# keurfonluu/stochopy

Measured on AMD Instinct MI355X. Metric: objective-fn evals/sec, higher is better.
Workload: dtype f64

## Files before the change

include/stochopy_hip.h:

```cpp
#ifndef STOCHOPY_HIP_H
#define STOCHOPY_HIP_H

#include <stdint.h>

#ifdef __cplusplus
extern "C" {
#endif

#define SX_ABI_VERSION 1

enum {
    SX_FUN_ACKLEY = 0,
    SX_FUN_GRIEWANK = 1,
    SX_FUN_QUARTIC = 2,
    SX_FUN_RASTRIGIN = 3,
    SX_FUN_ROSENBROCK = 4,
    SX_FUN_SPHERE = 5,
    SX_FUN_STYBLINSKI_TANG = 6,
    SX_FUN_COUNT = 7
};

enum { SX_DE_RAND1BIN = 0, SX_DE_RAND2BIN = 1, SX_DE_BEST1BIN = 2, SX_DE_BEST2BIN = 3 };

enum {
// ... 29 lines not shown
    int64_t gbidx;
    double gfit;
    double dx;
    int32_t status;
    int32_t done;
    int64_t reserved[3];
} sx_state;

typedef struct sx_de_args {
    double *buf0, *buf1;
    double *fit;
    double *candfit;
    double *gbest;
    const double *lower;
    const double *upper;
    sx_state *state;
    double *part_f;
    int64_t *part_i;
    const double *r1;
    const int32_t *donors;
    const int32_t *irand;
    const double *resample;
    int64_t P;
    int64_t ld;
    int64_t row0;
    int32_t n;
    int32_t fun_id;
    int32_t strategy;
    int32_t constraints;
    int32_t rng;
    int32_t maxiter;
    int32_t wide_from;
    int32_t pad;
    double F, CR, xtol, ftol;
    uint32_t key0, key1;
} sx_de_args;

int sx_de_generation(const sx_de_args *a, int finalize, void *stream);

int sx_select_finalize(const double *part_f, const int64_t *part_i, int64_t npart, const double *rows0,
                       const double *rows1, int64_t ld, int n, double *gbest, sx_state *state, int maxiter,
                       double xtol, double ftol, void *stream);

int sx_shard_best(const double *part_f, const int64_t *part_i, int64_t npart, const double *rows0,
                  const double *rows1, int64_t ld, int n, const sx_state *state, int64_t row0, double *record,
                  void *stream);
int sx_gather_finalize(const double *records, int world, int n, double *gbest, sx_state *state, int maxiter,
                       double xtol, double ftol, void *stream);
int sx_de_shard_generation(const struct sx_de_args *a, double *record, void *stream);

typedef struct sx_graph sx_graph;
int sx_de_graph_create(const sx_de_args *a, int ngen, sx_graph **out);
int sx_de_chain_launch(const sx_de_args *a, int parity, int finalize_only, void *stream);
int sx_de_chain_graph_create(const sx_de_args *a, int ngen, int start_parity, sx_graph **out);
int sx_graph_launch(sx_graph *g, void *stream);
int sx_graph_destroy(sx_graph *g);

#define SX_MAX_PEERS 8
#define SX_IPC_HANDLE_BYTES 64
typedef struct sx_xchg_args {
    uint64_t *peer[SX_MAX_PEERS];
    int32_t world, rank;
    int64_t timeout_ticks;
    int32_t *error;
    uint64_t *relay;
    const double *pop0[SX_MAX_PEERS];
    const double *pop1[SX_MAX_PEERS];
    int64_t global_rows, shard_rows;
} sx_xchg_args;
// ... 202 lines not shown
```

stochopy_amd/_lib.py:

```python
import ctypes as C
import os

_HERE = os.path.dirname(os.path.abspath(__file__))
LIB_PATH = os.path.join(_HERE, "lib", "libstochopy_hip.so")

SX_STATUS_NONE = 100
NARROW_DIM, WIDE_DIM = 4096, 262144


def wide_from():
    return int(lib().sx_wide_from())
SX_RNG_HOST, SX_RNG_PHILOX = 0, 1

FUN_IDS = {
    "ackley": 0,
    "griewank": 1,
    "quartic": 2,
    "rastrigin": 3,
    "rosenbrock": 4,
    "sphere": 5,
    "styblinski_tang": 6,
}
DE_STRATEGIES = {"rand1bin": 0, "rand2bin": 1, "best1bin": 2, "best2bin": 3}
DE_DONORS = {"rand1bin": 3, "rand2bin": 5, "best1bin": 2, "best2bin": 4}

vp = C.c_void_p
i64 = C.c_int64
i32 = C.c_int32
f64 = C.c_double


class SxState(C.Structure):
    _fields_ = [("it", i64), ("gbidx", i64), ("gfit", f64), ("dx", f64), ("status", i32), ("done", i32),
                ("reserved", i64 * 3)]


class SxDeArgs(C.Structure):
    _fields_ = [
        ("buf0", vp), ("buf1", vp), ("fit", vp), ("candfit", vp), ("gbest", vp), ("lower", vp),
        ("upper", vp), ("state", vp), ("part_f", vp), ("part_i", vp), ("r1", vp), ("donors", vp),
        ("irand", vp), ("resample", vp),
        ("P", i64), ("ld", i64), ("row0", i64),
        ("n", i32), ("fun_id", i32), ("strategy", i32), ("constraints", i32), ("rng", i32), ("maxiter", i32),
        ("wide_from", i32), ("pad", i32),
        ("F", f64), ("CR", f64), ("xtol", f64), ("ftol", f64),
        ("key0", C.c_uint32), ("key1", C.c_uint32),
    ]


class SxPsoArgs(C.Structure):
    _fields_ = [
        ("X", vp), ("V", vp), ("pbest", vp), ("pbestfit", vp), ("candfit", vp), ("gbest", vp), ("lower", vp),
        ("upper", vp), ("state", vp), ("part_f", vp), ("part_i", vp), ("r1", vp), ("r2", vp), ("pending_restart", vp),
        ("P", i64), ("ld", i64), ("row0", i64),
        ("n", i32), ("fun_id", i32), ("constraints", i32), ("rng", i32), ("maxiter", i32), ("pad", i32),
        ("w", f64), ("c1", f64), ("c2", f64), ("xtol", f64), ("ftol", f64),
        ("key0", C.c_uint32), ("key1", C.c_uint32),
    ]


SX_MAX_PEERS = 8
SX_IPC_HANDLE_BYTES = 64


class SxXchgArgs(C.Structure):
    _fields_ = [("peer", vp * SX_MAX_PEERS), ("world", i32), ("rank", i32), ("timeout_ticks", i64), ("error", vp),
                ("relay", vp), ("pop0", vp * SX_MAX_PEERS), ("pop1", vp * SX_MAX_PEERS), ("global_rows", i64),
                ("shard_rows", i64)]


class SxCmaState(C.Structure):
    _fields_ = [("it", i64), ("nfev", i64), ("best_row", i64), ("fbest", f64), ("sigma", f64), ("sigma_next", f64),
                ("tmp_coef", f64), ("psnorm", f64), ("status", i32), ("done", i32), ("stop_it", i64),
                ("reserved", f64 * 6)]


class SxVdArgs(C.Structure):
    _fields_ = [
        ("Z", vp), ("ary", vp), ("arx", vp), ("fit", vp), ("xmean", vp), ("xold", vp), ("dx", vp), ("dvec", vp),
        ("vvec", vp), ("vn", vp), ("pc", vp), ("zinj", vp), ("dy", vp), ("w", vp), ("mws", vp), ("mout", vp),
# ... 157 lines not shown
```

stochopy_amd/csrc/sx_de.hip:

```cpp
#define SX_DE_XM 0
#include "sx_de_kernel.hpp"
#include "sx_wide.hpp"

namespace sx {
void *de_chain_kernel(int fun_id, int n, int64_t P, int strategy, int constraints);
void *de_p2p_kernel(int fun_id, int n, int64_t P, int strategy, int constraints);
}

namespace {

int check_args(const sx_de_args *a) {
    SX_REQUIRE(a != nullptr, "sx_de: null args");
    SX_REQUIRE(a->buf0 && a->buf1 && a->fit && a->state && a->part_f && a->part_i, "sx_de: null device pointer");
    SX_REQUIRE(a->P >= 2 && a->P < (int64_t)1 << 31 && a->n >= 1 && a->ld >= a->n, "sx_de: bad shape");
    SX_REQUIRE(a->fun_id >= 0 && a->fun_id < SX_FUN_COUNT, "sx_de: unknown objective");
    SX_REQUIRE(a->strategy >= 0 && a->strategy <= 3, "sx_de: unknown strategy");
    SX_REQUIRE(a->P - 1 >= donors_of(a->strategy), "sx_de: popsize too small for the strategy");
    SX_REQUIRE(a->rng == SX_RNG_HOST || a->rng == SX_RNG_PHILOX, "sx_de: unknown rng mode");
    if (a->rng == SX_RNG_HOST) {
        SX_REQUIRE(a->r1 && a->donors && a->irand, "sx_de: host draws missing");
        SX_REQUIRE(a->constraints == 0 || a->resample, "sx_de: resample block missing");
    }
    SX_REQUIRE(a->constraints == 0 || (a->lower && a->upper), "sx_de: bounds missing");
    return 0;
}

de_kernel_t kernel_for(const sx_de_args *a) {
    return a->rng == SX_RNG_PHILOX ? pick_kernel<SX_RNG_PHILOX, 0>(a->fun_id, a->n, a->P, a->strategy, a->constraints)
                                   : pick_kernel<SX_RNG_HOST, 0>(a->fun_id, a->n, a->P, a->strategy, a->constraints);
}

Geometry geometry(const sx_de_args *a) {
    Geometry g = row_geometry(a->P, a->n, de_wide_from(a));
    if (!is_wide(a->n, de_wide_from(a))) g.lds = (size_t)rows_per_block(a->n) * gen_row_stride(a->n) * sizeof(double);
    return g;
}

}

extern "C" int sx_de_generation(const sx_de_args *a, int finalize, void *stream) {
    if (int rc = check_args(a)) return rc;
    hipStream_t s = (hipStream_t)stream;
    const Geometry g = geometry(a);
    if (is_wide(a->n, de_wide_from(a))) {
        if (int rc = wide_de_launch(a, s)) return rc;
    } else {
        PlanArg plan;
        if (make_plan_arg(a->fun_id, a->n, &plan)) return -1;
        hipLaunchKernelGGL(kernel_for(a), dim3(g.blocks), dim3(g.threads), g.lds, s, (const sx_state *)nullptr,
                           (const double *)nullptr, (const int64_t *)nullptr, (int64_t)g.blocks, *a, plan, 0, 0,
                           sx_xchg_args{});
        SX_LAUNCH_CHECK();
    }
    if (finalize) {
        SX_REQUIRE(a->gbest != nullptr, "sx_de_generation: the separate finalize kernel needs the gbest buffer");
        return sx_select_finalize(a->part_f, a->part_i, g.blocks, a->buf0, a->buf1, a->ld, a->n, a->gbest, a->state,
                                  a->maxiter, a->xtol, a->ftol, stream);
    }
    return 0;
}

extern "C" int sx_de_graph_create(const sx_de_args *a, int ngen, sx_graph **out) {
    if (int rc = check_args(a)) return rc;
    SX_REQUIRE(out != nullptr && ngen >= 1 && a->gbest != nullptr, "sx_de_graph_create: bad arguments");
    SX_REQUIRE(a->rng == SX_RNG_PHILOX, "sx_de_graph_create: graphs need in-kernel (Philox) draws");
    PlanArg plan = {};
    const bool wide = is_wide(a->n, de_wide_from(a));
    if (!wide && make_plan_arg(a->fun_id, a->n, &plan)) return -1;
    const Geometry g = geometry(a);
    sx_graph *gr = new sx_graph();
    SX_HIP(hipGraphCreate(&gr->graph, 0));
    sx_de_args args = *a;
    int zero = 0;
    int64_t npart = g.blocks;
    sx_xchg_args nox = {};
    const void *none = nullptr;
    void *kargs[] = {&none, &none, &none, &npart, &args, &plan, &zero, &zero, &nox};
    hipGraphNode_t prev = nullptr;
    for (int i = 0; i < ngen; ++i) {
        if (wide) {
            if (int rc = wide_de_add_node(gr->graph, &prev, a)) return rc;
        } else {
            hipKernelNodeParams kp = {};
            kp.func = (void *)kernel_for(a);
            kp.gridDim = dim3(g.blocks);
            kp.blockDim = dim3(g.threads);
            kp.sharedMemBytes = (unsigned)g.lds;
            kp.kernelParams = kargs;
            kp.extra = nullptr;
            hipGraphNode_t node;
            SX_HIP(hipGraphAddKernelNode(&node, gr->graph, prev ? &prev : nullptr, prev ? 1 : 0, &kp));
            prev = node;
        }
        if (int rc = add_finalize_node(gr->graph, &prev, a->part_f, a->part_i, g.blocks, a->buf0, a->buf1, a->ld, a->n,
                                       a->gbest, a->state, a->maxiter, a->xtol, a->ftol))
            return rc;
    }
    SX_HIP(hipGraphInstantiate(&gr->exec, gr->graph, nullptr, nullptr, 0));
    *out = gr;
    return 0;
}

extern "C" int sx_de_shard_generation(const sx_de_args *a, double *record, void *stream) {
    SX_REQUIRE(record != nullptr, "sx_de_shard_generation: null record");
    if (int rc = sx_de_generation(a, 0, stream)) return rc;
    return sx_shard_best(a->part_f, a->part_i, (int64_t)geometry(a).blocks, a->buf0, a->buf1, a->ld, a->n, a->state,
                         a->row0, record, stream);
}

static int check_chain(const sx_de_args *a, bool peer_exchange) {
    if (int rc = check_args(a)) return rc;
    SX_REQUIRE(a->rng == SX_RNG_PHILOX, "sx_de_chain: needs in-kernel (Philox) draws");
    SX_REQUIRE(!is_wide(a->n, de_wide_from(a)), "sx_de_chain: rows served by the one-workgroup-per-row kernels (n > wide_from) take the two-kernel path (sx_de_generation)");
    SX_REQUIRE(peer_exchange || geometry(a).blocks <= 512,
               "sx_de_chain: more than 512 workgroup records (use the two-kernel path)");
    return 0;
}

static int chain_launch(const sx_de_args *a, const sx_xchg_args *x, int parity, int finalize_only, void *stream) {
    if (int rc = check_chain(a, x != nullptr)) return rc;
    SX_REQUIRE(parity == 0 || parity == 1, "sx_de_chain_launch: parity must be 0 or 1");
    PlanArg plan;
    if (make_plan_arg(a->fun_id, a->n, &plan)) return -1;
    const Geometry g = geometry(a);
    de_kernel_t kern = (de_kernel_t)(x ? de_p2p_kernel(a->fun_id, a->n, a->P, a->strategy, a->constraints)
                                       : de_chain_kernel(a->fun_id, a->n, a->P, a->strategy, a->constraints));
    const unsigned blocks = finalize_only ? 1u : g.blocks + (x ? 1u : 0u);
    hipLaunchKernelGGL(kern, dim3(blocks), dim3(g.threads), g.lds, (hipStream_t)stream,
                       (const sx_state *)(a->state + parity), (const double *)(a->part_f + (int64_t)parity * g.blocks),
                       (const int64_t *)(a->part_i + (int64_t)parity * g.blocks), (int64_t)g.blocks, *a, plan, parity,
                       finalize_only ? 1 : 0, x ? *x : sx_xchg_args{});
    SX_LAUNCH_CHECK();
    return 0;
}

static int chain_graph_create(const sx_de_args *a, const sx_xchg_args *x, int ngen, int start_parity, sx_graph **out) {
    if (int rc = check_chain(a, x != nullptr)) return rc;
    SX_REQUIRE(out != nullptr && ngen >= 1 && (start_parity == 0 || start_parity == 1),
               "sx_de_chain_graph_create: bad arguments");
    PlanArg plan;
    if (make_plan_arg(a->fun_id, a->n, &plan)) return -1;
    const Geometry g = geometry(a);
    sx_graph *gr = new sx_graph();
    SX_HIP(hipGraphCreate(&gr->graph, 0));
    sx_de_args args = *a;
    sx_xchg_args xa = x ? *x : sx_xchg_args{};
    int mode = 0;
    int64_t npart = g.blocks;
    hipGraphNode_t prev = nullptr;
    for (int i = 0; i < ngen; ++i) {
        int parity = (start_parity + i) & 1;
        const sx_state *sin_pre = a->state + parity;
        const double *pf_pre = a->part_f + (int64_t)parity * npart;
        const int64_t *pi_pre = a->part_i + (int64_t)parity * npart;
        void *kargs[] = {&sin_pre, &pf_pre, &pi_pre, &npart, &args, &plan, &parity, &mode, &xa};
        hipKernelNodeParams kp = {};
        kp.func = x ? de_p2p_kernel(a->fun_id, a->n, a->P, a->strategy, a->constraints)
                    : de_chain_kernel(a->fun_id, a->n, a->P, a->strategy, a->constraints);
        kp.gridDim = dim3(g.blocks + (x ? 1u : 0u));
        kp.blockDim = dim3(g.threads);
        kp.sharedMemBytes = (unsigned)g.lds;
        kp.kernelParams = kargs;
        kp.extra = nullptr;
        hipGraphNode_t node;
        SX_HIP(hipGraphAddKernelNode(&node, gr->graph, prev ? &prev : nullptr, prev ? 1 : 0, &kp));
        prev = node;
    }
    SX_HIP(hipGraphInstantiate(&gr->exec, gr->graph, nullptr, nullptr, 0));
    *out = gr;
    return 0;
}

extern "C" int sx_de_chain_launch(const sx_de_args *a, int parity, int finalize_only, void *stream) {
    return chain_launch(a, nullptr, parity, finalize_only, stream);
}
extern "C" int sx_de_chain_graph_create(const sx_de_args *a, int ngen, int start_parity, sx_graph **out) {
    return chain_graph_create(a, nullptr, ngen, start_parity, out);
}

extern "C" int sx_de_p2p_launch(const sx_de_args *a, const sx_xchg_args *x, int parity, int finalize_only,
                                void *stream) {
    if (int rc = check_xchg_args(x)) return rc;
    return chain_launch(a, x, parity, finalize_only, stream);
}
extern "C" int sx_de_p2p_graph_create(const sx_de_args *a, const sx_xchg_args *x, int ngen, int start_parity,
                                      sx_graph **out) {
    if (int rc = check_xchg_args(x)) return rc;
    return chain_graph_create(a, x, ngen, start_parity, out);
// ... 17 lines not shown
```

stochopy_amd/csrc/sx_de_kernel.hpp:

```cpp
#pragma once
#ifndef SX_DE_XM
#error "define SX_DE_XM (0, 1 or 2) before including sx_de_kernel.hpp"
#endif
#include <type_traits>
#include <vector>

#include "sx_device.hpp"
#include "sx_host.hpp"
#include "sx_rowops.hpp"
#include "sx_xchg.hpp"

namespace sx {
int make_plan_arg(int fun_id, int n, PlanArg *out);
int add_finalize_node(hipGraph_t graph, hipGraphNode_t *prev, const double *part_f, const int64_t *part_i,
                      int64_t npart, const double *rows0, const double *rows1, int64_t ld, int n, double *gbest,
                      sx_state *state, int maxiter, double xtol, double ftol);
int check_xchg_args(const sx_xchg_args *x);
}
using namespace sx;

#if defined(SX_TRACE) && SX_DE_XM == 1
__device__ unsigned long long sx_trace_buf[1024 * 16];
#define SX_TP(k)                                                                              \
    do {                                                                                      \
// ... 103 lines not shown
                        break;
                    }
                    w[u] = ll_load(src + j);
                }
                __hip_atomic_store(dst + j, w[u], __ATOMIC_RELAXED, __HIP_MEMORY_SCOPE_AGENT);
            }
        }
        __builtin_amdgcn_fence(__ATOMIC_RELEASE, "agent");
        __syncthreads();
        if (threadIdx.x == 0)
            __hip_atomic_store(dst + xchg_slot_words(a.n), (uint64_t)tag, __ATOMIC_RELEASE, __HIP_MEMORY_SCOPE_AGENT);
        if (wave != 0) return;
    }
    if (lane == 0) {
        int status = SX_STATUS_NONE;
        if (it >= 2) {
            if (gf <= a.ftol)
                status = 1;
            else if (it >= a.maxiter)
                status = -1;
        }
        sx_state *so = a.state + (mode == 1 ? 2 : 1 - chain_p);
        so->it = it;
        so->gbidx = gi;
        so->gfit = gf;
        so->dx = 0.0;
        so->status = status;
        so->done = status != SX_STATUS_NONE;
        so->reserved[0] = prev_winner;
        so->reserved[1] = winner;
    }
}

constexpr int kStep = 4;

#ifndef SX_DE_NFIX_WAVES
#define SX_DE_NFIX_WAVES 1
#endif
#ifndef SX_DE_WAVE_ROWS_WAVES
#define SX_DE_WAVE_ROWS_WAVES 1
#endif
template <int FUN, int RNG, int XM, int LPR, bool FULL, int NFIX = 0, int STRAT = -1, bool ONEB = false>
__global__ __launch_bounds__(kMaxWavesPerBlock *kWave, (NFIX != 0 && XM <= 1) ? SX_DE_NFIX_WAVES
                                                       : (NFIX == 0 && XM == 0 && STRAT >= 0 && LPR == kWave) ? SX_DE_WAVE_ROWS_WAVES
                                                                                                                 : 1) void de_generation_kernel(const sx_state *const sin_pre,
                                                                                 const double *const pf_pre,
                                                                                 const int64_t *const pi_pre,
                                                                                 const int64_t npart,
                                                                                 const sx_de_args a,
                                                                                 const PlanArg plan,
                                                                                 const int chain_p, const int mode,
                                                                                 const sx_xchg_args x) {
    constexpr bool CHAIN = XM >= 1;
    constexpr bool P2P = XM == 2;
    extern __shared__ __attribute__((aligned(16))) double lds[];
    __shared__ double sf[kMaxRowsPerBlock];
    __shared__ int64_t si[kMaxRowsPerBlock];
    __shared__ double s_gf;
    __shared__ int64_t s_gi;
    __shared__ int s_winner;
    SX_TP(0);
    const int n = NFIX ? NFIX : a.n;
    const int64_t P = a.P, ld = a.ld;
    const RowIds<LPR> id(P, P2P ? 1 : 0);
    const int l = id.l;
    const int64_t rowc = id.rowc;
    double *U = lds + id.slot * gen_row_stride(n);

    const sx_state *sin = (CHAIN && !P2P) ? sin_pre : CHAIN ? a.state + chain_p : a.state;
    constexpr int kRecPerLane = 8;
    double pfv[kRecPerLane];
    using rec_t = typename std::conditional<LPR == kWave, int32_t, int64_t>::type;
    constexpr rec_t kNoRec = LPR == kWave ? (rec_t)INT32_MAX : (rec_t)INT64_MAX;
    rec_t piv[kRecPerLane];
#ifndef SX_CHAIN_REC_WAVE0
#define SX_CHAIN_REC_WAVE0 1
#endif
    if (CHAIN && !P2P && (!SX_CHAIN_REC_WAVE0 || id.wave == 0)) {
        const double *pf = pf_pre;
        const int64_t *pi = pi_pre;
        const int per = (int)((npart + kWave - 1) / kWave);
        const int64_t k0 = (int64_t)id.lane * per;
#pragma unroll
        for (int u = 0; u < kRecPerLane; ++u) {
            const bool in = u < per && k0 + u < npart;
            pfv[u] = in ? pf[k0 + u] : __builtin_huge_val();
            piv[u] = in ? (rec_t)pi[k0 + u] : kNoRec;
        }
    }
    if (P2P && blockIdx.x == 0) {
        p2p_service(a, x, chain_p, mode, npart, sin, LPR == kWave);
        return;
    }
    if (sin->done) {
        if (CHAIN && mode == 1 && threadIdx.x == 0) a.state[2] = *sin;
        return;
    }
    const int64_t it = CHAIN ? sin->it + 1 : sin->it;
    SX_TP(6);

    const uint32_t gen = (uint32_t)(it + 1);
    const double *__restrict__ cur = (it & 1) ? a.buf1 : a.buf0;
    double *__restrict__ nxt = (it & 1) ? a.buf0 : a.buf1;
    const double fold = a.fit[rowc];
    const double *__restrict__ xi = cur + rowc * ld;
    const uint32_t grow = (uint32_t)(a.row0 + rowc);
    const int strategy = STRAT >= 0 ? STRAT : a.strategy;
    const int k = donors_of(strategy);
    const bool repair = STRAT >= 0 ? false : a.constraints != 0;
    const bool use_best = strategy == SX_DE_BEST1BIN || strategy == SX_DE_BEST2BIN;

    int64_t d[kMaxDonors];
    int irand;
    const bool gdon = P2P && x.global_rows > 0;
    if (RNG == SX_RNG_PHILOX) {
        philox_donors(gdon ? x.global_rows : P, k, gdon ? a.row0 + rowc : rowc, grow, gen, a.key0, a.key1, n, d, irand);
    } else {
#pragma unroll
        for (int t = 0; t < kMaxDonors; ++t) d[t] = t < k ? (int64_t)a.donors[(int64_t)t * P + rowc] : 0;
        irand = a.irand[rowc];
    }
    SX_TP(1);
    const double *pd[kMaxDonors];
#pragma unroll
    for (int t = 0; t < kMaxDonors; ++t) pd[t] = cur + d[t] * ld;
    if (gdon) {
#pragma unroll
        for (int t = 0; t < kMaxDonors; ++t) {
            const int owner = (int)(d[t] / x.shard_rows);
            const int64_t lrow = d[t] - (int64_t)owner * x.shard_rows;
            const double *base = nullptr;
#pragma unroll
            for (int r = 0; r < SX_MAX_PEERS; ++r)
                if (r == owner) base = (it & 1) ? x.pop1[r] : x.pop0[r];
            pd[t] = base + lrow * ld;
        }
    }
    const double F = a.F, CR = a.CR;
    const double *r1row = RNG == SX_RNG_HOST ? a.r1 + rowc * (int64_t)n : nullptr;
    const double *rsrow = (RNG == SX_RNG_HOST && repair) ? a.resample + rowc * (int64_t)n : nullptr;

    struct Batch {
        double x[kStep], d[kMaxDonors][kStep], r[kStep], rs[kStep];
    };
    Batch B0;
    auto load_batch = [&](int q0, Batch &bt) {
        double(&bx)[kStep] = bt.x;
        double(&bd)[kMaxDonors][kStep] = bt.d;
        double(&br)[kStep] = bt.r;
        double(&brs)[kStep] = bt.rs;
#pragma unroll
        for (int t = 0; t < kStep; ++t) {
            const int e = (q0 + t) * LPR + l;
            const bool in = FULL || e < n;
            bx[t] = in ? xi[e] : 0.0;
#pragma unroll
            for (int s = 0; s < kMaxDonors; ++s) {
                if (P2P && gdon)
// ... 1 lines not shown
                                             : 0.0;
                else
                    bd[s][t] = (s < k && in) ? pd[s][e] : 0.0;
            }
            br[t] = 2.0;
            brs[t] = 0.0;
            if (RNG == SX_RNG_HOST && in) {
                br[t] = r1row[e];
                if (repair) brs[t] = rsrow[e];
            }
        }
        if (RNG == SX_RNG_PHILOX) {
#pragma unroll
            for (int t = 0; t < kStep; t += 2) {
                const U4 w = philox4x32_10((uint32_t)((q0 + t) >> 1) * (uint32_t)LPR + (uint32_t)l, grow, gen, kPurposeDeCross,
                                           a.key0, a.key1);
                br[t] = u53(w.x, w.y);
                br[t + 1] = u53(w.z, w.w);
            }
            if (repair) {
#pragma unroll
                for (int t = 0; t < kStep; ++t) {
                    const int e = (q0 + t) * LPR + l;
                    if (FULL || e < n)
                        brs[t] = a.lower[e] + (a.upper[e] - a.lower[e]) *
                                                  philox_u53(e, LPR, grow, gen, kPurposeDeResample, a.key0, a.key1);
                }
            }
        }
    };
    if (!gdon) load_batch(0, B0);

    int64_t gbidx = 0;
    double *part_f_out = a.part_f;
    int64_t *part_i_out = a.part_i;
    const uint32_t xtag = (uint32_t)(it + 1);
    const uint64_t *gbw = nullptr;
    if (P2P) {
        const uint64_t *rel = x.relay + (int64_t)chain_p * xchg_relay_stride(n);
        if (id.wave == 0) {
            double bf;
            int64_t bi;
            int winner;
            bool ok = __atomic_load_n(x.error, __ATOMIC_RELAXED) == 0 &&
                      xchg_wait_best(x.peer[x.rank] + xchg_slot_offset(n, chain_p, 0), n, x.world, xtag,
                                     x.timeout_ticks, id.lane, bf, bi, winner);
            if (ok && LPR == kWave && use_best && !(it >= 2 && (bf <= a.ftol || it >= a.maxiter))) {
                const uint64_t t0 = wall_clock64();
                while (__hip_atomic_load(rel + xchg_slot_words(n), __ATOMIC_RELAXED, __HIP_MEMORY_SCOPE_AGENT) !=
                       (uint64_t)xtag) {
                    if ((int64_t)(wall_clock64() - t0) > x.timeout_ticks) {
                        ok = false;
                        break;
                    }
                    __builtin_amdgcn_s_sleep(2);
                }
            }
            if (id.lane == 0) {
                s_gf = bf;
                s_gi = bi;
                s_winner = ok ? winner : -1;
                if (!ok) atomicExch(x.error, 1);
            }
        }
        __syncthreads();
        const int winner = s_winner;
        if (winner < 0) return;
        const double bf = s_gf;
        const int64_t bi = s_gi;
        if (it >= 2 && (bf <= a.ftol || it >= a.maxiter)) return;
        gbidx = bi;
        gbw = LPR == kWave ? rel + 4 : x.peer[x.rank] + xchg_slot_offset(n, chain_p, winner) + 4;
        part_f_out = a.part_f + (int64_t)(1 - chain_p) * npart;
        part_i_out = a.part_i + (int64_t)(1 - chain_p) * npart;
        if (gdon) load_batch(0, B0);
    } else if (CHAIN) {
        double bf = 0.0;
        int64_t bi = 0;
        if (!SX_CHAIN_REC_WAVE0 || id.wave == 0) {
        double lm[kRecPerLane / 2];
#pragma unroll
        for (int u = 0; u < kRecPerLane / 2; ++u) lm[u] = fmin(pfv[2 * u], pfv[2 * u + 1]);
        const double lmin = fmin(fmin(lm[0], lm[1]), fmin(lm[2], lm[3]));
        bf = wave_min_f64(lmin);
        rec_t br = piv[0];
        double bv = pfv[0];
#pragma unroll
        for (int u = kRecPerLane - 1; u >= 0; --u)
            if (pfv[u] == bf) br = piv[u], bv = pfv[u];
        unsigned long long hit = __ballot(lmin == bf);
        bool lnan = false;
#pragma unroll
        for (int u = 0; u < kRecPerLane; ++u) lnan |= is_nan(pfv[u]);
        const unsigned long long nanl = __ballot(lnan);
        if (nanl) {
            hit = nanl;
#pragma unroll
            for (int u = kRecPerLane - 1; u >= 0; --u)
                if (is_nan(pfv[u])) br = piv[u], bv = pfv[u];
        }
        const int src = hit ? (int)__ffsll((long long)hit) - 1 : 0;
        bf = readlane_f64(bv, src);
        if (LPR == kWave) {
            bi = (int64_t)__builtin_amdgcn_readlane((int)br, src);
        } else {
            const int lo = __builtin_amdgcn_readlane((int)((int64_t)br & 0xffffffffll), src);
            const int hi = __builtin_amdgcn_readlane((int)((int64_t)br >> 32), src);
            bi = ((int64_t)hi << 32) | (int64_t)(unsigned)lo;
        }
        }
        if (SX_CHAIN_REC_WAVE0) {
            if (id.wave == 0 && id.lane == 0) s_gf = bf, s_gi = bi;
            __syncthreads();
            bf = s_gf, bi = s_gi;
        }
        int status = SX_STATUS_NONE;
        if (it >= 2) {
            if (bf <= a.ftol)
                status = 1;
            else if (it >= a.maxiter)
                status = -1;
        }
        if (blockIdx.x == 0 && threadIdx.x == 0) {
            sx_state *so = a.state + (mode == 1 ? 2 : 1 - chain_p);
            so->it = it;
            so->gbidx = bi;
            so->gfit = bf;
            so->dx = 0.0;
            so->status = status;
            so->done = status != SX_STATUS_NONE;
            so->reserved[0] = sin->gbidx;
        }
        if (status != SX_STATUS_NONE || mode == 1) return;
        gbidx = bi;
        part_f_out = a.part_f + (int64_t)(1 - chain_p) * npart;
        part_i_out = a.part_i + (int64_t)(1 - chain_p) * npart;
    } else {
        gbidx = sin->gbidx;
    }
    const double *__restrict__ gb = P2P ? cur : a.gbest != nullptr ? a.gbest : cur + gbidx * ld;

    const int nq = (n + LPR - 1) / LPR;
    constexpr bool kRegRow = NFIX != 0 || LPR < kWave || ONEB;
    double keep[kStep];
    auto trial_batch = [&](int q0, const Batch &bt) {
        const double(&bx)[kStep] = bt.x;
        const double(&bd)[kMaxDonors][kStep] = bt.d;
        const double(&br)[kStep] = bt.r;
        const double(&brs)[kStep] = bt.rs;
        double g[kStep];
        if (P2P) {
            if (use_best) {
                const uint64_t t0 = wall_clock64();
                for (int attempt = 0;; ++attempt) {
                    uint64_t lo[kStep], hi[kStep];
                    bool ok = true;
                    const bool cached = LPR == kWave && attempt == 0;
#pragma unroll
                    for (int t = 0; t < kStep; ++t) {
                        const int e = (q0 + t) * LPR + l;
                        const bool in = FULL || e < n;
                        if (cached) {
                            const ulonglong2 w2 =
                                in ? *reinterpret_cast<const ulonglong2 *>(gbw + 2 * e) : make_ulonglong2(0, 0);
                            lo[t] = w2.x;
                            hi[t] = w2.y;
                        } else if (LPR == kWave) {
                            lo[t] = in ? __hip_atomic_load(gbw + 2 * e, __ATOMIC_RELAXED, __HIP_MEMORY_SCOPE_AGENT) : 0;
                            hi[t] = in ? __hip_atomic_load(gbw + 2 * e + 1, __ATOMIC_RELAXED, __HIP_MEMORY_SCOPE_AGENT) : 0;
                        } else {
                            lo[t] = in ? ll_load(gbw + 2 * e) : 0;
                            hi[t] = in ? ll_load(gbw + 2 * e + 1) : 0;
                        }
// ... 19 lines not shown
            for (int t = 0; t < kStep; ++t) {
                const int e = (q0 + t) * LPR + l;
                g[t] = (use_best && (FULL || e < n)) ? gb[e] : 0.0;
            }
        }
#pragma unroll
        for (int t = 0; t < kStep; ++t) {
            const int e = (q0 + t) * LPR + l;
            if (FULL || e < n) {
                const double v = de_mutant(strategy, g[t], bd[0][t], bd[1][t], bd[2][t], bd[3][t], bd[4][t], F);
                double cand = (e == irand || br[t] <= CR) ? v : bx[t];
                if (repair && (cand < a.lower[e] || cand > a.upper[e])) cand = brs[t];
                U[e] = cand;
                if (kRegRow) keep[t] = cand;
            }
        }
    };
    if constexpr (LPR < kWave) {
        trial_batch(0, B0);
    } else {
        trial_batch(0, B0);
        if constexpr (!ONEB) {
            for (int q0 = kStep; q0 < nq; q0 += kStep) {
                load_batch(q0, B0);
                trial_batch(q0, B0);
            }
        }
    }

    SX_TP(2);
    const double fc = row_objective<FUN, LPR, FULL, NFIX, SX_LONG_STATIC, ONEB>(U, n, plan, l);
    SX_TP(3);
    const bool better = fc < fold;
    if (FULL || id.active) {
        double *__restrict__ xo = nxt + id.row * ld;
        if constexpr (kRegRow) {
#pragma unroll
            for (int t = 0; t < kStep; ++t)
                if (NFIX != 0 || l + t * LPR < n) st_stream(xo + l + t * LPR, better ? keep[t] : B0.x[t]);
        } else {
            const double *__restrict__ src = better ? U : xi;
            for (int e0 = l; e0 < n; e0 += kStep * LPR) {
                double v[kStep];
#pragma unroll
                for (int t = 0; t < kStep; ++t) v[t] = (FULL || e0 + t * LPR < n) ? src[e0 + t * LPR] : 0.0;
#pragma unroll
                for (int t = 0; t < kStep; ++t)
                    if (FULL || e0 + t * LPR < n) xo[e0 + t * LPR] = v[t];
            }
        }
        if (l == 0) {
            if (better) a.fit[id.row] = fc;
            if (a.candfit != nullptr) a.candfit[id.row] = fc;
        }
    }
    SX_TP(4);
    block_partial<LPR>(better ? fc : fold, id, sf, si, part_f_out, part_i_out);
    SX_TP(5);
}

typedef void (*de_kernel_t)(const sx_state *, const double *, const int64_t *, const int64_t, const sx_de_args,
                            const PlanArg, const int, const int, const sx_xchg_args);

template <int RNG, int XM, int LPR, bool FULL, int NFIX = 0, int STRAT = -1, bool ONEB = false>
de_kernel_t pick_kernel_lpr(int fun_id) {
    constexpr bool SPECIAL = STRAT != -1 || ONEB || NFIX != 0;
    switch (fun_id) {
        case SX_FUN_ACKLEY: return de_generation_kernel<SX_FUN_ACKLEY, RNG, XM, LPR, FULL, NFIX, STRAT, ONEB>;
        case SX_FUN_RASTRIGIN: return de_generation_kernel<SX_FUN_RASTRIGIN, RNG, XM, LPR, FULL, NFIX, STRAT, ONEB>;
        case SX_FUN_ROSENBROCK: return de_generation_kernel<SX_FUN_ROSENBROCK, RNG, XM, LPR, FULL, NFIX, STRAT, ONEB>;
        case SX_FUN_SPHERE: return de_generation_kernel<SX_FUN_SPHERE, RNG, XM, LPR, FULL, NFIX, STRAT, ONEB>;
    }
    if constexpr (!SPECIAL) {
        switch (fun_id) {
            case SX_FUN_GRIEWANK: return de_generation_kernel<SX_FUN_GRIEWANK, RNG, XM, LPR, FULL, NFIX, STRAT, ONEB>;
            case SX_FUN_QUARTIC: return de_generation_kernel<SX_FUN_QUARTIC, RNG, XM, LPR, FULL, NFIX, STRAT, ONEB>;
            case SX_FUN_STYBLINSKI_TANG: return de_generation_kernel<SX_FUN_STYBLINSKI_TANG, RNG, XM, LPR, FULL, NFIX, STRAT, ONEB>;
        }
    }
    return nullptr;
}

template <int RNG, int XM, int LPR, bool FULL, int NFIX>
de_kernel_t pick_kernel_fixed(int fun_id, int strategy, int constraints) {
    if constexpr (XM == 2 && LPR != 32) {
        return pick_kernel_lpr<RNG, XM, LPR, FULL, NFIX>(fun_id);
    } else {
        if (constraints != 0 || !hot_objective(fun_id)) return pick_kernel_lpr<RNG, XM, LPR, FULL, NFIX>(fun_id);
        switch (strategy) {
            case SX_DE_RAND1BIN: return pick_kernel_lpr<RNG, XM, LPR, FULL, NFIX, NFIX ? SX_DE_RAND1BIN : -1>(fun_id);
            case SX_DE_BEST1BIN: return pick_kernel_lpr<RNG, XM, LPR, FULL, NFIX, NFIX ? SX_DE_BEST1BIN : -1>(fun_id);
        }
        return pick_kernel_lpr<RNG, XM, LPR, FULL, NFIX>(fun_id);
    }
// ... 39 lines not shown
```

stochopy_amd/optimize/_de.py:

```python
import ctypes as C
import os
import warnings

import numpy as np

from .. import _device, _lib, _rng
from . import _common
from ._helpers import register
from ._population import _PopulationRun

__all__ = ["minimize"]


def minimize(
    fun,
    bounds,
    x0=None,
    args=(),
    maxiter=100,
    popsize=10,
    mutation=0.5,
    recombination=0.9,
    strategy="best1bin",
    seed=None,
    xtol=1.0e-8,
    ftol=1.0e-8,
    constraints=None,
    updating="immediate",
    workers=1,
    backend=None,
    return_all=False,
    verbosity=1.0,
    callback=None,
    rng=None,
    exchange=None,
    donors=None,
    strict_updating=None,
    host_workers=None,
    host_backend=None,
):
    fun_id = _common.resolve_objective(fun, args, workers, backend, host_workers, host_backend)
    lower, upper = _common.as_bounds(bounds)
    if x0 is not None:
        if np.ndim(x0) != 2 or np.shape(x0)[1] != len(bounds):
# ... 197 lines not shown
        while ngen >= self.GRAPH_CHUNK:
            if self._graph is None:
                g = C.c_void_p()
                _lib.check(ctx.L.sx_de_graph_create(C.byref(self.args), self.GRAPH_CHUNK, C.byref(g)),
                           "sx_de_graph_create")
                self._graph = g
            _lib.check(ctx.L.sx_graph_launch(self._graph, ctx.stream_ptr), "sx_graph_launch")
            ngen -= self.GRAPH_CHUNK
        for _ in range(ngen):
            _lib.check(ctx.L.sx_de_generation(C.byref(self.args), 1, ctx.stream_ptr), "sx_de_generation")

    def _setup(self):
        ctx, P, n = self.ctx, self.P, self.n
        t = _device.torch()
        self.stream = _rng.make_init_stream(self.rng, self.seed)
        d_bounds = ctx.upload_async(np.concatenate([self.lower, self.upper]))
        self.d_lower, self.d_upper = d_bounds[:n], d_bounds[n:]
        if self.global_donors:
            self.bufs = list(self.px.share_population(P, n, self.Ptotal))
        else:
            self.bufs = [ctx.empty((P, n)), ctx.empty((P, n))]
        if self.x0 is None and self.rng == "philox":
            _rng.philox_latin_hypercube(ctx, self.bufs[1], self.row0, self.Ptotal, self.d_lower, self.d_upper, self.seed)
        else:
            if self.x0 is not None:
                X0 = np.array(self.x0, dtype=np.float64)
            else:
                X0 = self.stream.latin_hypercube(self.Ptotal, n, self.lower, self.upper)
            if self.world is not None:
                X0 = np.ascontiguousarray(X0[self.row0 : self.row0 + P])
            self.bufs[1].copy_(ctx.upload(X0))
        self.fit = ctx.empty((P,))
        self.candfit = ctx.empty((P,))
        npart = self.npart
        self.part_f = ctx.empty((npart,))
        self.part_i = ctx.empty((npart,), dtype=t.int64)
        _common.evaluate_rows(ctx, self.fun_id, self.bufs[1], n, self.fit)
        self.candfit.copy_(self.fit)
        quiet_start = (self.chain and self.world is None and self.px is None and self.callback is None
                       and not self.return_all and self.external is None)
        if quiet_start:
            rec_f = t.full((2, npart), float("inf"), dtype=t.float64, device=ctx.device)
            rec_i = t.full((2, npart), np.iinfo(np.int64).max, dtype=t.int64, device=ctx.device)
            _lib.check(ctx.L.sx_argmin(_device.ptr(self.fit), P, _device.ptr(self.part_f), _device.ptr(self.part_i),
                                       npart, _device.ptr(rec_i), _device.ptr(rec_f), ctx.stream_ptr), "sx_argmin")
            g, gfit0 = 0, 0.0
            self.gbest = None
        else:
            out_i = ctx.empty((1,), dtype=t.int64)
            out_f = ctx.empty((1,))
            _lib.check(ctx.L.sx_argmin(_device.ptr(self.fit), P, _device.ptr(self.part_f), _device.ptr(self.part_i),
                                       npart, _device.ptr(out_i), _device.ptr(out_f), ctx.stream_ptr), "sx_argmin")
            g = int(out_i.cpu()[0])
            gfit0 = float(out_f.cpu()[0])
            self.gbest = self.bufs[1][g].clone()
        if self.world is not None and self.px is None:
            from ..parallel import best_of_records

            self.record = ctx.empty((n + 2,))
            self.records = ctx.empty((self.world.size, n + 2))
            self.record[0] = gfit0
            self.record[1] = float(self.row0 + g)
            self.record[2:].copy_(self.gbest)
            self.world.all_gather_records(self.record, self.records)
            wbest, gfit0, g = best_of_records(self.records.cpu().numpy())
            self.gbest.copy_(self.records[wbest, 2:])
        st = _lib.SxState(it=1, gbidx=g, gfit=gfit0, dx=0.0, status=_lib.SX_STATUS_NONE, done=0)
        if self.chain:
            s0 = _lib.SxState(it=0, gbidx=g, gfit=gfit0, dx=0.0, status=_lib.SX_STATUS_NONE, done=0)
            raw = np.frombuffer(bytes(s0) + bytes(st) + bytes(st), dtype=np.int64).copy()
            self.state = ctx.upload_async(raw)
            if quiet_start:
                self.part_f, self.part_i = rec_f, rec_i
            else:
                pf = np.full((2, npart), np.inf)
                pi = np.full((2, npart), np.iinfo(np.int64).max, dtype=np.int64)
                pf[0, 0], pi[0, 0] = gfit0, g
                self.part_f = ctx.upload(pf)
                self.part_i = ctx.upload(pi)
        else:
            self.state = ctx.upload(np.frombuffer(bytes(st), dtype=np.int64).copy())
        key0, key1 = _rng.philox_key(self.seed) if self.rng == "philox" else (0, 0)
        a = _lib.SxDeArgs()
        a.buf0, a.buf1 = self.bufs[0].data_ptr(), self.bufs[1].data_ptr()
        if self.immediate:
            a.buf0 = a.buf1
        a.fit, a.candfit = self.fit.data_ptr(), self.candfit.data_ptr()
        a.lower, a.upper, a.state = self.d_lower.data_ptr(), self.d_upper.data_ptr(), self.state.data_ptr()
        a.part_f, a.part_i = self.part_f.data_ptr(), self.part_i.data_ptr()
        a.gbest = None if self.chain else self.gbest.data_ptr()
        a.P, a.ld, a.row0, a.n = P, n, self.row0, n
        a.wide_from = self.wide_from
        a.fun_id, a.strategy = (self.fun_id if self.external is None else 0), _lib.DE_STRATEGIES[self.strategy]
        if self.external is not None:
            self.cand = ctx.empty((P, n))
            self.cand_f = ctx.empty((P,))
        self.it_enq = 1
        a.constraints = 1 if self.constraints == "Random" else 0
        a.rng = _lib.SX_RNG_PHILOX if self.rng == "philox" else _lib.SX_RNG_HOST
        a.maxiter = self.maxiter
        a.F, a.CR, a.xtol, a.ftol = self.F, self.CR, self.xtol, self.ftol
        a.key0, a.key1 = key0, key1
        self.args = a
        if self.rng == "numpy-legacy":
            self.h_r1 = t.empty((P, n), dtype=t.float64).pin_memory()
            self.h_don = t.empty((self.k, P), dtype=t.int32).pin_memory()
            self.h_irand = t.empty((P,), dtype=t.int32).pin_memory()
            self.d_r1 = ctx.empty((P, n))
            self.d_don = ctx.empty((self.k, P), dtype=t.int32)
            self.d_irand = ctx.empty((P,), dtype=t.int32)
            a.r1, a.donors, a.irand = self.d_r1.data_ptr(), self.d_don.data_ptr(), self.d_irand.data_ptr()
            if a.constraints:
                self.h_rs = t.empty((P, n), dtype=t.float64).pin_memory()
                self.d_rs = ctx.empty((P, n))
                a.resample = self.d_rs.data_ptr()
        self.st = st
        if self.world is not None and (self.return_all or self.callback is not None):
            self.Xfull = ctx.empty((self.Ptotal, n))
            self.candfull = ctx.empty((self.Ptotal,))
            if self.px is not None:
                st = self.read_state()
                self.gbest.copy_(ctx.upload(self._best_row(st)))
        if self.return_all:
            self.nout = int(np.ceil(self.verbosity * self.Ptotal))
            rows = max(self.nout, 1)
            self.xall = ctx.empty((self.maxiter, rows, n))
            self.funall = ctx.empty((self.maxiter, rows))
            if self.nout > 0:
                X1, f1 = self._whole_population(1)
                self.xall[0].copy_(X1[: self.nout])
                self.funall[0].copy_(f1[: self.nout])
            else:
                self.xall[0, 0].copy_(self.gbest if self.world is not None else self.bufs[1][g])
                self.funall[0, 0] = st.gfit
        self.st = st

    def _population(self, it):
        return self.bufs[1] if self.immediate else self.bufs[it & 1]

    def _best_row(self, st):
        if self.px is not None:
            return self.px.read_record((st.it - 1) & 1, int(st.reserved[1]))[2]
        if self.chain:
            return self._population(st.it)[st.gbidx].cpu().numpy()
        return self.gbest.cpu().numpy()

    def _settle_status(self, st):
        status = int(st.status)
        if self.chain and status == 1:
            if self.px is not None:
                prev = self.px.read_record(st.it & 1, int(st.reserved[0]))[2]
            else:
                prev = self._population(st.it - 1)[st.reserved[0]].cpu().numpy()
            if np.linalg.norm(prev - self._best_row(st)) <= self.xtol:
                status = 0
        return status

    def _host_draws(self):
        s = self.stream
        s.random(None, out=self.h_r1.numpy())
        if self.immediate:
            rs = self.h_rs.numpy() if self.args.constraints else None
            s.de_async_draws(self.P, self.k, self.n, self.h_don.numpy(), self.h_irand.numpy(), self.lower, self.upper, rs)
            self.d_r1.copy_(self.h_r1, non_blocking=True)
            self.d_don.copy_(self.h_don, non_blocking=True)
            self.d_irand.copy_(self.h_irand, non_blocking=True)
            if rs is not None:
                self.d_rs.copy_(self.h_rs, non_blocking=True)
            return
        s.de_donors(self.P, self.k, out=self.h_don.numpy())
        self.h_irand.numpy()[:] = s.randint(self.n, self.P)
        self.d_r1.copy_(self.h_r1, non_blocking=True)
        self.d_don.copy_(self.h_don, non_blocking=True)
        self.d_irand.copy_(self.h_irand, non_blocking=True)
        if self.args.constraints:
            s.uniform_rows(self.lower, self.upper, self.P, out=self.h_rs.numpy())
            self.d_rs.copy_(self.h_rs, non_blocking=True)

    def _external_generation(self):
        ctx, L, p, n = self.ctx, self.ctx.L, _device.ptr, self.n
        it = self.it_enq
        _lib.check(L.sx_de_propose(C.byref(self.args), p(self.cand), ctx.stream_ptr), "sx_de_propose")
        self.cand_f.copy_(self.external(ctx, self.cand))
        cur, nxt = self.bufs[it & 1], self.bufs[(it + 1) & 1]
        _lib.check(L.sx_rows_select(p(self.cand), n, p(self.cand_f), p(cur), p(nxt), n, p(self.fit), p(self.candfit),
                                    self.P, n, p(self.state), p(self.part_f), p(self.part_i), ctx.stream_ptr),
# ... 90 lines not shown
```

Baseline: 605.3 million.

## Track per-row buffer ownership with a bitmap to skip rewriting losing trial rows

In the single-GPU chained DE kernel, each row now has a bit in a double-buffered row map that records which of the two population buffers holds its current vector. Only rows whose trial vector improves get written to the other buffer, and then their bit flips. Rows that lose are no longer copied forward, which cuts global write traffic in each generation. In exchange every donor and best-row read first looks up the bitmap staged in LDS, adds a ballot and map store per block, and makes the host-side population reads more involved.

```diff
diff --git a/include/stochopy_hip.h b/include/stochopy_hip.h
--- a/include/stochopy_hip.h
+++ b/include/stochopy_hip.h
@@ -85,9 +85,11 @@
     int32_t maxiter;
     int32_t wide_from;
     int32_t pad;
+    uint32_t *rowmap;
     double F, CR, xtol, ftol;
     uint32_t key0, key1;
 } sx_de_args;
+#define SX_DE_ROWMAP_WORDS 256
 
 int sx_de_generation(const sx_de_args *a, int finalize, void *stream);
 
diff --git a/stochopy_amd/_lib.py b/stochopy_amd/_lib.py
--- a/stochopy_amd/_lib.py
+++ b/stochopy_amd/_lib.py
@@ -42,10 +42,13 @@
         ("irand", vp), ("resample", vp),
         ("P", i64), ("ld", i64), ("row0", i64),
         ("n", i32), ("fun_id", i32), ("strategy", i32), ("constraints", i32), ("rng", i32), ("maxiter", i32),
-        ("wide_from", i32), ("pad", i32),
+        ("wide_from", i32), ("pad", i32), ("rowmap", vp),
         ("F", f64), ("CR", f64), ("xtol", f64), ("ftol", f64),
         ("key0", C.c_uint32), ("key1", C.c_uint32),
     ]
+
+
+DE_ROWMAP_WORDS = 256
 
 
 class SxPsoArgs(C.Structure):
diff --git a/stochopy_amd/csrc/sx_de.hip b/stochopy_amd/csrc/sx_de.hip
--- a/stochopy_amd/csrc/sx_de.hip
+++ b/stochopy_amd/csrc/sx_de.hip
@@ -48,8 +48,8 @@
         PlanArg plan;
         if (make_plan_arg(a->fun_id, a->n, &plan)) return -1;
         hipLaunchKernelGGL(kernel_for(a), dim3(g.blocks), dim3(g.threads), g.lds, s, (const sx_state *)nullptr,
-                           (const double *)nullptr, (const int64_t *)nullptr, (int64_t)g.blocks, *a, plan, 0, 0,
-                           sx_xchg_args{});
+                           (const double *)nullptr, (const int64_t *)nullptr, (int64_t)g.blocks, (const uint32_t *)nullptr,
+                           *a, plan, 0, 0, sx_xchg_args{});
         SX_LAUNCH_CHECK();
     }
     if (finalize) {
@@ -75,7 +75,7 @@
     int64_t npart = g.blocks;
     sx_xchg_args nox = {};
     const void *none = nullptr;
-    void *kargs[] = {&none, &none, &none, &npart, &args, &plan, &zero, &zero, &nox};
+    void *kargs[] = {&none, &none, &none, &npart, &none, &args, &plan, &zero, &zero, &nox};
     hipGraphNode_t prev = nullptr;
     for (int i = 0; i < ngen; ++i) {
         if (wide) {
@@ -114,6 +114,7 @@
     SX_REQUIRE(!is_wide(a->n, de_wide_from(a)), "sx_de_chain: rows served by the one-workgroup-per-row kernels (n > wide_from) take the two-kernel path (sx_de_generation)");
     SX_REQUIRE(peer_exchange || geometry(a).blocks <= 512,
                "sx_de_chain: more than 512 workgroup records (use the two-kernel path)");
+    SX_REQUIRE(peer_exchange || a->rowmap != nullptr, "sx_de_chain: the single-GPU chained kernel needs the row map (rowmap)");
     return 0;
 }
 
@@ -128,7 +129,8 @@
     const unsigned blocks = finalize_only ? 1u : g.blocks + (x ? 1u : 0u);
     hipLaunchKernelGGL(kern, dim3(blocks), dim3(g.threads), g.lds, (hipStream_t)stream,
                        (const sx_state *)(a->state + parity), (const double *)(a->part_f + (int64_t)parity * g.blocks),
-                       (const int64_t *)(a->part_i + (int64_t)parity * g.blocks), (int64_t)g.blocks, *a, plan, parity,
+                       (const int64_t *)(a->part_i + (int64_t)parity * g.blocks), (int64_t)g.blocks,
+                       (const uint32_t *)(x ? nullptr : a->rowmap + parity * SX_DE_ROWMAP_WORDS), *a, plan, parity,
                        finalize_only ? 1 : 0, x ? *x : sx_xchg_args{});
     SX_LAUNCH_CHECK();
     return 0;
@@ -153,7 +155,8 @@
         const sx_state *sin_pre = a->state + parity;
         const double *pf_pre = a->part_f + (int64_t)parity * npart;
         const int64_t *pi_pre = a->part_i + (int64_t)parity * npart;
-        void *kargs[] = {&sin_pre, &pf_pre, &pi_pre, &npart, &args, &plan, &parity, &mode, &xa};
+        const uint32_t *map_pre = x ? nullptr : a->rowmap + parity * SX_DE_ROWMAP_WORDS;
+        void *kargs[] = {&sin_pre, &pf_pre, &pi_pre, &npart, &map_pre, &args, &plan, &parity, &mode, &xa};
         hipKernelNodeParams kp = {};
         kp.func = x ? de_p2p_kernel(a->fun_id, a->n, a->P, a->strategy, a->constraints)
                     : de_chain_kernel(a->fun_id, a->n, a->P, a->strategy, a->constraints);
diff --git a/stochopy_amd/csrc/sx_de_kernel.hpp b/stochopy_amd/csrc/sx_de_kernel.hpp
--- a/stochopy_amd/csrc/sx_de_kernel.hpp
+++ b/stochopy_amd/csrc/sx_de_kernel.hpp
@@ -159,6 +159,20 @@
     }
 }
 
+static_assert(kMaxRowsPerBlock <= 16 && SX_DE_ROWMAP_WORDS * 32 >= 512 * kMaxRowsPerBlock, "row map: 512 records of <= 16 rows");
+__device__ __forceinline__ uint32_t rowmap_bit(const uint32_t *map, int64_t r) { return (map[r >> 5] >> (r & 31)) & 1u; }
+__device__ __forceinline__ void rowmap_store(uint32_t *map, int64_t r0, int rows, uint32_t bits) {
+    if (rows == 16) {
+        reinterpret_cast<uint16_t *>(map)[r0 >> 4] = (uint16_t)bits;
+    } else if (rows == 8) {
+        reinterpret_cast<uint8_t *>(map)[r0 >> 3] = (uint8_t)bits;
+    } else {
+        const uint32_t mask = ((1u << rows) - 1u) << (r0 & 31);
+        atomicAnd(map + (r0 >> 5), ~mask);
+        atomicOr(map + (r0 >> 5), (bits << (r0 & 31)) & mask);
+    }
+}
+
 constexpr int kStep = 4;
 
 #ifndef SX_DE_NFIX_WAVES
@@ -174,18 +188,23 @@
                                                                                  const double *const pf_pre,
                                                                                  const int64_t *const pi_pre,
                                                                                  const int64_t npart,
+                                                                                 const uint32_t *const map_pre,
                                                                                  const sx_de_args a,
                                                                                  const PlanArg plan,
                                                                                  const int chain_p, const int mode,
                                                                                  const sx_xchg_args x) {
     constexpr bool CHAIN = XM >= 1;
     constexpr bool P2P = XM == 2;
+    constexpr bool MAP = XM == 1;
     extern __shared__ __attribute__((aligned(16))) double lds[];
     __shared__ double sf[kMaxRowsPerBlock];
     __shared__ int64_t si[kMaxRowsPerBlock];
     __shared__ double s_gf;
     __shared__ int64_t s_gi;
     __shared__ int s_winner;
+    __shared__ uint32_t s_gbit;
+    __shared__ uint32_t s_bit[kMaxRowsPerBlock];
+    __shared__ __attribute__((aligned(16))) uint32_t s_map[MAP ? kMaxWavesPerBlock : 1][MAP ? SX_DE_ROWMAP_WORDS : 4];
     SX_TP(0);
     const int n = NFIX ? NFIX : a.n;
     const int64_t P = a.P, ld = a.ld;
@@ -215,6 +234,10 @@
             piv[u] = in ? (rec_t)pi[k0 + u] : kNoRec;
         }
     }
+    const bool map_lane = MAP && (int64_t)id.lane * 8 < npart;
+    uint4 map_in = {0u, 0u, 0u, 0u};
+    if (map_lane) map_in = reinterpret_cast<const uint4 *>(map_pre)[id.lane];
+    const uint32_t *wmap = s_map[MAP ? id.wave : 0];
     if (P2P && blockIdx.x == 0) {
         p2p_service(a, x, chain_p, mode, npart, sin, LPR == kWave);
         return;
@@ -224,13 +247,20 @@
         return;
     }
     const int64_t it = CHAIN ? sin->it + 1 : sin->it;
+    if (map_lane) reinterpret_cast<uint4 *>(s_map[id.wave])[id.lane] = map_in;
+    if (MAP) lds_wave_fence();
     SX_TP(6);
 
     const uint32_t gen = (uint32_t)(it + 1);
     const double *__restrict__ cur = (it & 1) ? a.buf1 : a.buf0;
     double *__restrict__ nxt = (it & 1) ? a.buf0 : a.buf1;
     const double fold = a.fit[rowc];
-    const double *__restrict__ xi = cur + rowc * ld;
+    auto row_bit = [&](int64_t r) -> uint32_t {
+        const uint32_t b = rowmap_bit(wmap, r);
+        return LPR == kWave ? (uint32_t)__builtin_amdgcn_readfirstlane((int)b) : b;
+    };
+    const uint32_t obit = MAP ? row_bit(rowc) : 0u;
+    const double *__restrict__ xi = (MAP ? (obit ? a.buf1 : a.buf0) : cur) + rowc * ld;
     const uint32_t grow = (uint32_t)(a.row0 + rowc);
     const int strategy = STRAT >= 0 ? STRAT : a.strategy;
     const int k = donors_of(strategy);
@@ -250,7 +280,8 @@
     SX_TP(1);
     const double *pd[kMaxDonors];
 #pragma unroll
-    for (int t = 0; t < kMaxDonors; ++t) pd[t] = cur + d[t] * ld;
+    for (int t = 0; t < kMaxDonors; ++t)
+        pd[t] = (MAP && t < k ? (row_bit(d[t]) ? a.buf1 : a.buf0) : cur) + d[t] * ld;
     if (gdon) {
 #pragma unroll
         for (int t = 0; t < kMaxDonors; ++t) {
@@ -318,6 +349,7 @@
     if (!gdon) load_batch(0, B0);
 
     int64_t gbidx = 0;
+    const double *gbuf = cur;
     double *part_f_out = a.part_f;
     int64_t *part_i_out = a.part_i;
     const uint32_t xtag = (uint32_t)(it + 1);
@@ -363,6 +395,7 @@
     } else if (CHAIN) {
         double bf = 0.0;
         int64_t bi = 0;
+        uint32_t gbit = 0;
         if (!SX_CHAIN_REC_WAVE0 || id.wave == 0) {
         double lm[kRecPerLane / 2];
 #pragma unroll
@@ -394,11 +427,16 @@
             const int hi = __builtin_amdgcn_readlane((int)((int64_t)br >> 32), src);
             bi = ((int64_t)hi << 32) | (int64_t)(unsigned)lo;
         }
+        if (MAP) gbit = rowmap_bit(wmap, bi);
         }
         if (SX_CHAIN_REC_WAVE0) {
-            if (id.wave == 0 && id.lane == 0) s_gf = bf, s_gi = bi;
+            if (id.wave == 0 && id.lane == 0) {
+                s_gf = bf, s_gi = bi;
+                if (MAP) s_gbit = gbit;
+            }
             __syncthreads();
             bf = s_gf, bi = s_gi;
+            if (MAP) gbit = s_gbit;
         }
         int status = SX_STATUS_NONE;
         if (it >= 2) {
@@ -419,12 +457,13 @@
         }
         if (status != SX_STATUS_NONE || mode == 1) return;
         gbidx = bi;
+        gbuf = gbit ? a.buf1 : a.buf0;
         part_f_out = a.part_f + (int64_t)(1 - chain_p) * npart;
         part_i_out = a.part_i + (int64_t)(1 - chain_p) * npart;
     } else {
         gbidx = sin->gbidx;
     }
-    const double *__restrict__ gb = P2P ? cur : a.gbest != nullptr ? a.gbest : cur + gbidx * ld;
+    const double *__restrict__ gb = P2P ? cur : a.gbest != nullptr ? a.gbest : gbuf + gbidx * ld;
 
     const int nq = (n + LPR - 1) / LPR;
     constexpr bool kRegRow = NFIX != 0 || LPR < kWave || ONEB;
@@ -510,9 +549,27 @@
     const double fc = row_objective<FUN, LPR, FULL, NFIX, SX_LONG_STATIC, ONEB>(U, n, plan, l);
     SX_TP(3);
     const bool better = fc < fold;
+    if (MAP && l == 0) s_bit[id.slot] = obit ^ (better ? 1u : 0u);
     if (FULL || id.active) {
-        double *__restrict__ xo = nxt + id.row * ld;
-        if constexpr (kRegRow) {
+        double *__restrict__ xo = (MAP ? (obit ? a.buf0 : a.buf1) : nxt) + id.row * ld;
+        if constexpr (MAP) {
+            if (better) {
+                if constexpr (kRegRow) {
+#pragma unroll
+                    for (int t = 0; t < kStep; ++t)
+                        if (NFIX != 0 || l + t * LPR < n) st_stream(xo + l + t * LPR, keep[t]);
+                } else {
+                    for (int e0 = l; e0 < n; e0 += kStep * LPR) {
+                        double v[kStep];
+#pragma unroll
+                        for (int t = 0; t < kStep; ++t) v[t] = (FULL || e0 + t * LPR < n) ? U[e0 + t * LPR] : 0.0;
+#pragma unroll
+                        for (int t = 0; t < kStep; ++t)
+                            if (FULL || e0 + t * LPR < n) xo[e0 + t * LPR] = v[t];
+                    }
+                }
+            }
+        } else if constexpr (kRegRow) {
 #pragma unroll
             for (int t = 0; t < kStep; ++t)
                 if (NFIX != 0 || l + t * LPR < n) st_stream(xo + l + t * LPR, better ? keep[t] : B0.x[t]);
@@ -534,10 +591,15 @@
     }
     SX_TP(4);
     block_partial<LPR>(better ? fc : fold, id, sf, si, part_f_out, part_i_out);
+    if (MAP && threadIdx.x < kWave) {
+        const int rows = (int)(blockDim.x >> 6) * RowIds<LPR>::RPW;
+        const uint32_t bits = (uint32_t)__ballot((int)threadIdx.x < rows && s_bit[threadIdx.x] != 0u);
+        if (threadIdx.x == 0) rowmap_store(a.rowmap + (1 - chain_p) * SX_DE_ROWMAP_WORDS, (int64_t)id.block * rows, rows, bits);
+    }
     SX_TP(5);
 }
 
-typedef void (*de_kernel_t)(const sx_state *, const double *, const int64_t *, const int64_t, const sx_de_args,
+typedef void (*de_kernel_t)(const sx_state *, const double *, const int64_t *, const int64_t, const uint32_t *, const sx_de_args,
                             const PlanArg, const int, const int, const sx_xchg_args);
 
 template <int RNG, int XM, int LPR, bool FULL, int NFIX = 0, int STRAT = -1, bool ONEB = false>
diff --git a/stochopy_amd/optimize/_de.py b/stochopy_amd/optimize/_de.py
--- a/stochopy_amd/optimize/_de.py
+++ b/stochopy_amd/optimize/_de.py
@@ -10,6 +10,16 @@
 from ._population import _PopulationRun
 
 __all__ = ["minimize"]
+
+
+def rowmap_slot(it):
+    return 1 - (it & 1)
+
+
+def rowmap_rows(words, P):
+    t = _device.torch()
+    shifts = t.arange(32, dtype=t.int32, device=words.device)
+    return ((words[:, None] >> shifts) & 1).reshape(-1)[:P].bool()
 
 
 def minimize(
@@ -273,6 +283,9 @@
             self.bufs[1].copy_(ctx.upload(X0))
         self.fit = ctx.empty((P,))
         self.candfit = ctx.empty((P,))
+        self.rowmap = None
+        if self.chain and self.px is None:
+            self.rowmap = t.full((2, _lib.DE_ROWMAP_WORDS), -1, dtype=t.int32, device=ctx.device)
         npart = self.npart
         self.part_f = ctx.empty((npart,))
         self.part_i = ctx.empty((npart,), dtype=t.int64)
@@ -330,6 +343,7 @@
         a.lower, a.upper, a.state = self.d_lower.data_ptr(), self.d_upper.data_ptr(), self.state.data_ptr()
         a.part_f, a.part_i = self.part_f.data_ptr(), self.part_i.data_ptr()
         a.gbest = None if self.chain else self.gbest.data_ptr()
+        a.rowmap = None if self.rowmap is None else self.rowmap.data_ptr()
         a.P, a.ld, a.row0, a.n = P, n, self.row0, n
         a.wide_from = self.wide_from
         a.fun_id, a.strategy = (self.fun_id if self.external is None else 0), _lib.DE_STRATEGIES[self.strategy]
@@ -377,13 +391,24 @@
         self.st = st
 
     def _population(self, it):
+        if self.rowmap is not None:
+            t = _device.torch()
+            return t.where(rowmap_rows(self.rowmap[rowmap_slot(it)], self.P)[:, None], self.bufs[1], self.bufs[0])
         return self.bufs[1] if self.immediate else self.bufs[it & 1]
+
+    def _row(self, it, r):
+        r = int(r)
+        if self.rowmap is not None:
+            t = _device.torch()
+            bit = (self.rowmap[rowmap_slot(it), r >> 5] >> (r & 31)) & 1
+            return t.where(bit.bool(), self.bufs[1][r], self.bufs[0][r]).cpu().numpy()
+        return self._population(it)[r].cpu().numpy()
 
     def _best_row(self, st):
         if self.px is not None:
             return self.px.read_record((st.it - 1) & 1, int(st.reserved[1]))[2]
         if self.chain:
-            return self._population(st.it)[st.gbidx].cpu().numpy()
+            return self._row(st.it, st.gbidx)
         return self.gbest.cpu().numpy()
 
     def _settle_status(self, st):
@@ -392,7 +417,7 @@
             if self.px is not None:
                 prev = self.px.read_record(st.it & 1, int(st.reserved[0]))[2]
             else:
-                prev = self._population(st.it - 1)[st.reserved[0]].cpu().numpy()
+                prev = self._row(st.it - 1, st.reserved[0])
             if np.linalg.norm(prev - self._best_row(st)) <= self.xtol:
                 status = 0
         return status
```

Result: slower. 576.3 million (median of 6 runs) (-4.8%).
